# GBATZOLIS/conditional_score_diffusion

Hardware: AMD Instinct MI355X
Metric: images/sec for 1000-step PC sampling, ddpm_paired_SR3 score net of celebA_SR3_160 (BASELINE configs[1]), 160x160 (higher is better)
Workload: dtype f16x3 (every operand carried as hi + lo fp16 = 22 significand bits, 3 MFMAs per product, f32 accumulate; f32-class: the per-op test tolerance is the f32 kernel's, network error 1.9e-6 vs the reference); 1 GPU; BASELINE configs[1]: celebA_SR3_160 (ddpm_paired_SR3, nf=96, ch_mult (1,1,2,2,3,3), attn 20/10/5), 1000-step PC (reverse_diffusion + langevin, snr 0.15), batch 64 per GPU, random-init weights, synthetic LR inputs; images_per_gpu=64, global_batch=64, noise=on-device Philox4x32-10, precision_mode=fp16x3

## Files before the change

conditional_score_diffusion_amd/_lib.py:

```python
import ctypes
import os
import subprocess
import sys

_HERE = os.path.dirname(os.path.abspath(__file__))
LIB_PATH = os.environ.get('CSD_LIB_PATH', os.path.join(_HERE, 'libcsd_hip.so'))
CSRC = os.path.join(_HERE, 'csrc')

MAX_LEVELS = 8
MAX_ATTN = 8

ACT_IDS = {'none': 0, 'swish': 1, 'relu': 2, 'lrelu': 3, 'elu': 4}
PREC_IDS = {'fp32': 0, 'f32': 0, 'fp16x3': 1, 'fp16': 2, 'fp16f8': 3}


class UNetConfig(ctypes.Structure):
    _fields_ = [('arch', ctypes.c_int32), ('nf', ctypes.c_int32), ('n_levels', ctypes.c_int32),
                ('ch_mult', ctypes.c_int32 * MAX_LEVELS), ('num_res_blocks', ctypes.c_int32),
                ('n_attn', ctypes.c_int32), ('attn_resolutions', ctypes.c_int32 * MAX_ATTN),
                ('image_size', ctypes.c_int32), ('x_channels', ctypes.c_int32),
                ('y_channels', ctypes.c_int32), ('out_channels', ctypes.c_int32),
                ('resamp_with_conv', ctypes.c_int32), ('conditional', ctypes.c_int32),
                ('centered', ctypes.c_int32), ('act', ctypes.c_int32), ('precision', ctypes.c_int32),
                ('skip_rescale', ctypes.c_int32), ('progressive', ctypes.c_int32), ('progressive_input', ctypes.c_int32),
# ... 86 lines not shown
    'csd_fused_bias_act': (_i, [_vp, _vp, _vp, _vp, _i64, _i, _i64, _i, _i, _f, _f, _vp]),
    'csd_nearest_up2': (_i, [_vp, _vp, _i, _i, _i, _i, _vp]),
    'csd_timestep_embedding': (_i, [_vp, _vp, _i, _i, _vp]),
    'csd_conv_wgrad_scratch_bytes': (_sz, [_i, _i, _i, _i, _i, _i, _i, _i]),
    'csd_conv2d_wgrad': (_i, [_vp, _vp, _vp, _i, _i, _i, _i, _i, _i, _i, _i, _i, _vp, _vp]),
    'csd_groupnorm_act_backward': (_i, [_vp, _vp, _vp, _vp, _vp, _vp, _vp, _i, _i, _i, _i, _i, _f, _i, _vp]),
    'csd_attention_backward_scratch_bytes': (_sz, [_i, _i, _i, _i]),
    'csd_attention_backward': (_i, [_vp, _vp, _vp, _vp, _vp, _vp, _vp, _i, _i, _i, _i, _vp, _vp]),
    'csd_bgemm': (_i, [_vp, _vp, _vp, _i, _i, _i, _i64, _i64, _i64, _i64, _i64, _i64, _i, _i64, _i64, _i64, _f, _vp]),
    'csd_sum_inner': (_i, [_vp, _vp, _i64, _i64, _vp]),
    'csd_sum_rows': (_i, [_vp, _vp, _i, _i, _vp]),
    'csd_act': (_i, [_vp, _vp, _vp, _i, _i64, _vp]),
    'csd_mul': (_i, [_vp, _vp, _vp, _i64, _vp]),
    'csd_conv3x3_block_scratch_bytes': (_sz, [_i, _i]),
    'csd_conv3x3_block': (_i, [_vp, _vp, _vp, _vp, _vp, _vp, _vp, _i, _vp, _f, _vp, _vp, _i, _i, _i, _i, _i, _i, _i, _vp, _vp]),
    'csd_conv2d_ex': (_i, [_vp, _vp, _vp, _vp, _i, _i, _i, _i, _i, _i, _i, _i, _i, _i, _i, _vp, _vp]),
    'csd_conv2d_wgrad_ex': (_i, [_vp, _vp, _vp, _i, _i, _i, _i, _i, _i, _i, _i, _i, _i, _vp, _vp]),
    'csd_groupnorm_nhwc_scratch_bytes': (_sz, [_i, _i, _i]),
    'csd_groupnorm_act_nhwc': (_i, [_vp, _vp, _vp, _vp, _vp, _vp, _i, _i, _i, _i, _f, _i, _vp, _vp]),
    'csd_groupnorm_act_backward_nhwc': (_i, [_vp, _vp, _vp, _vp, _vp, _vp, _vp, _vp, _vp, _i, _i, _i, _i, _i, _i, _vp, _vp]),
    'csd_bias_add_nhwc': (_i, [_vp, _vp, _vp, _i, _i, _i, _vp]),
    'csd_sum_pixels_scratch_bytes': (_sz, [_i, _i, _i]),
    'csd_sum_pixels_nhwc': (_i, [_vp, _vp, _i, _i, _i, _vp, _vp]),
    'csd_zero_insert_odd_nhwc': (_i, [_vp, _vp, _i, _i, _i, _i, _vp]),
    'csd_sumpool2_nhwc': (_i, [_vp, _vp, _i, _i, _i, _i, _vp]),
    'csd_attention_nhwc': (_i, [_vp, _vp, _i, _i, _i, _vp]),
    'csd_attention_nhwc_prec': (_i, [_vp, _vp, _i, _i, _i, _i, _vp]),
    'csd_attention_backward_nhwc': (_i, [_vp, _vp, _vp, _i, _i, _i, _vp, _vp]),
    'csd_adam_step': (_i, [_vp, _vp, _vp, _vp, _vp, _vp, _i64, _i, _f, _f, _f, _f, _f, _f, _f, _vp]),
    'csd_global_norm_scratch_bytes': (_sz, []),
# ... 81 lines not shown
```

conditional_score_diffusion_amd/csrc/common.h:

```cpp
#pragma once
#include <hip/hip_runtime.h>
#include <stdint.h>
#include <stdio.h>
#include <string>

#include "../../include/csd.h"

#ifdef CSD_TUNE
#define CSD_TUNE_ENV(name) getenv(name)
#else
#define CSD_TUNE_ENV(name) (static_cast<const char*>(nullptr))
#endif

namespace csd {

void set_error(const char* fmt, ...);
const char* get_error();

#define CSD_CHECK_HIP(expr)                                                         \
  do {                                                                              \
    hipError_t _e = (expr);                                                         \
    if (_e != hipSuccess) {                                                         \
      csd::set_error("%s:%d: %s -> %s", __FILE__, __LINE__, #expr, hipGetErrorString(_e)); \
      return CSD_ERR_HIP;                                                           \
// ... 119 lines not shown
int conv16_plan_tiles(ConvPlan* p, int ns, int kcs = 1, bool lc = false);
size_t conv16_packed_bytes(const ConvPlan& p, int ns);
int conv16_pack_weight(const ConvPlan& p, int ns, const float* w, int layout, int cin_src, int cout_src,
                       int cout_off, void* wpack, hipStream_t s);
int conv16_launch(const ConvPlan& p, int ns, const ConvArgs& a, hipStream_t s, bool in16 = false);
bool conv16q_supported(const ConvPlan& p, int ns);
size_t conv16q_packed_bytes(const ConvPlan& p, int ns);
int conv16q_pack_weight(const ConvPlan& p, int ns, const float* w, int layout, int cin_src, int cout_src, int cout_off,
                        void* wpack, hipStream_t s);
int conv16q_plan_tiles(ConvPlan* p, int ns);
bool conv16q_up4_supported(const ConvPlan& p, int ns);
bool conv16q_up4_stats_ok(const ConvPlan& p);
size_t conv16q_up4_packed_bytes(const ConvPlan& p, int ns);
int conv16q_pack_weight_up4(const ConvPlan& p, int ns, const float* w, void* wpack, hipStream_t s);
int conv16q_launch(const ConvPlan& p, int ns, const ConvArgs& a, hipStream_t s, bool raw = false);
bool convff_supported(const ConvPlan& p, int ns);
size_t convff_packed_bytes(const ConvPlan& p, int ns);
int convff_pack_weight(const ConvPlan& p, int ns, const float* w, int layout, int cin_src, int cout_src, int cout_off,
                       void* wpack, hipStream_t s);
int convff_plan_tiles(ConvPlan* p, int ns);
bool convff_pipelined(const ConvPlan& p, int ns);
int convff_launch(const ConvPlan& p, int ns, const ConvArgs& a, hipStream_t s);
bool pw16_supported(const ConvPlan& p, int ns);
size_t pw16_packed_bytes(const ConvPlan& p, int ns);
int pw16_pack_weight(const ConvPlan& p, int ns, const float* w, int layout, int cin_src, int cout_src, int cout_off,
                     void* wpack, hipStream_t s);
int pw16_launch(const ConvPlan& p, int ns, const ConvArgs& a, hipStream_t s);
bool pw16_taps_supported(int cin, int cout, int ns);
int pw16_taps_cout(int cout);
int pw16_pack_weight_taps(const ConvPlan& p, int ns, const float* w, int cout, void* wpack, hipStream_t s);
// ... 103 lines not shown
```

conditional_score_diffusion_amd/csrc/conv_f16_q.hip:

```cpp
#include <stdlib.h>
#include <type_traits>

#include "conv_f16_kernel.h"

namespace csd {

typedef float floatx4q __attribute__((ext_vector_type(4)));
typedef unsigned int uint4q __attribute__((ext_vector_type(4)));

#define C16Q_THREADS 256

__device__ __forceinline__ double dpp_row16_sum(double v) {
#define CSD_DPP_STEP(CTRL)                                                                                   \
  {                                                                                                          \
    const int lo = __builtin_amdgcn_mov_dpp(__double2loint(v), CTRL, 0xF, 0xF, true);                        \
    const int hi = __builtin_amdgcn_mov_dpp(__double2hiint(v), CTRL, 0xF, 0xF, true);                        \
    v += __hiloint2double(hi, lo);                                                                           \
  }
  CSD_DPP_STEP(0xB1)
  CSD_DPP_STEP(0x4E)
  CSD_DPP_STEP(0x124)
  CSD_DPP_STEP(0x128)
#undef CSD_DPP_STEP
  return v;
}
__device__ __forceinline__ float dpp_row16_sum(float v) {
#define CSD_DPP_STEP_F(CTRL) v += __int_as_float(__builtin_amdgcn_mov_dpp(__float_as_int(v), CTRL, 0xF, 0xF, true));
  CSD_DPP_STEP_F(0xB1)
  CSD_DPP_STEP_F(0x4E)
  CSD_DPP_STEP_F(0x124)
  CSD_DPP_STEP_F(0x128)
#undef CSD_DPP_STEP_F
  return v;
}

typedef int int8q __attribute__((ext_vector_type(8)));

template <int MQ, int NS, bool MASK, int PWC, int S, int NTQ, bool F8, bool UP4 = false, bool RAW = false>
__global__ __launch_bounds__(C16Q_THREADS, 2) void conv_f16_q_kernel(const void* __restrict__ g_hi,
                                                                    const void* __restrict__ g_lo,
                                                                    const char* __restrict__ g_wpack,
                                                                    const Conv16KArgs k) {
  static_assert(!UP4 || (S == 1 && !F8), "the phase form is the stride-1 Upsample conv (a resampling conv: full split)");
  static_assert(!RAW || (NS == 2 && !F8), "the fp32-source form splits into two fp16 planes");
  constexpr int TAPS = UP4 ? 4 : 9, KS = UP4 ? 2 : 3, KCS = 2;
  constexpr int LO = 32 * KCS;
  constexpr int PSB = 32 * KCS * NS + 16;
  constexpr int NPIX = 2 * MQ * 16;
  constexpr int SPP = 2 * NS * KCS;
  constexpr int NU0 = (S == 2) ? ((NS == 2) ? 10 : 5) : ((NS == 2) ? 7 : 4);
  constexpr int NU = RAW ? 2 * ((NU0 + 1) / 2) : NU0;
  constexpr int rstride = PWC * PSB;
  constexpr int WSTEP = NTQ * NS * 1024;
  constexpr int GC = 32 * NTQ, HC = 16 * NTQ;
  extern __shared__ __attribute__((aligned(16))) char smem16[];

  const int tid = threadIdx.x;
#ifdef CSD_C16_TIMING
  int ts_n = 0;
#define Q_TSTAMP() do { if (k.a.dbg && tid == 0 && blockIdx.x < 4095 && ts_n < 8) k.a.dbg[blockIdx.x * 8 + ts_n++] = clock64(); } while (0)
#else
#define Q_TSTAMP() do { } while (0)
#endif
  Q_TSTAMP();
  const int lane = tid & 63;
  const int wave = __builtin_amdgcn_readfirstlane(tid >> 6);
  const int mi = wave >> 1, ni = wave & 1;
// ... 5 lines not shown
    const int xcd = bid & 7, slot = bid >> 3;
    const int q = nb >> 3, r = nb & 7;
    w = (xcd < r ? xcd * (q + 1) : r * (q + 1) + (xcd - r) * q) + slot;
  }
  const int ng = w % k.n_groups;
  const int tile4 = w / k.n_groups;
  const int ph = UP4 ? (tile4 & 3) : 0, pa = ph >> 1, pb = ph & 1;
  const int tile = UP4 ? (tile4 >> 2) : tile4;
  const int tile_y = tile / k.tiles_x;
  const int ov0 = tile_y * k.TH, ox0 = (tile - tile_y * k.tiles_x) * k.TW;
  const int Py = UP4 ? 1 - pa : ((S == 2) ? 0 : 1), Px = UP4 ? 1 - pb : ((S == 2) ? 0 : 1);
  const int prow0 = ov0 * S - Py, pcol0 = ox0 * S - Px;
  const int EH = (S == 2) ? k.IH : k.OH, EW = (S == 2) ? k.IW : k.OW;
  const int Cin = k.C0;
  const int npatch = k.PH * k.PW;
  const int patch_bytes = k.PH * PWC * PSB;
  int* const otab = reinterpret_cast<int*>(smem16 + patch_bytes);
  int* const btab = otab + NPIX;
  int* const vtab = btab + NPIX;
  int* const stab = vtab + NPIX;
  int* const dtab = stab + npatch;

  for (int m = tid; m < NPIX; m += C16Q_THREADS) {
    const int ty = m / k.TW, tx = m - ty * k.TW;
    const int ov = ov0 + ty, ox = ox0 + tx;
    const bool mv = (m < k.TH * k.TW) && (ov < k.B * k.OH) && (ox < k.OW);
    const int b = ov / k.OH, oy = ov - b * k.OH;
    unsigned vb = 0;
#pragma unroll
    for (int r = 0; r < KS; ++r) {
      const int iy = oy * S + r - Py, ix = ox * S + r - Px;
      vb |= ((mv && iy >= 0 && iy < EH) ? 1u : 0u) << r;
      vb |= ((mv && ix >= 0 && ix < EW) ? 1u : 0u) << (3 + r);
    }
    otab[m] = mv ? (UP4 ? (ov - ov0) * 4 * k.OW + 2 * ox : (ov - ov0) * k.OW + ox) : -1;
    btab[m] = mv ? b : 0;
    vtab[m] = (int)vb;
  }
  for (int pix = tid; pix < npatch; pix += C16Q_THREADS) {
    const int pr = pix / k.PW, pc = pix - pr * k.PW;
    const int vr = prow0 + pr, col = pcol0 + pc;
    const int img_lo = MASK ? 0 : (ov0 / k.OH) * EH;
    const int img_hi = MASK ? k.B * EH : img_lo + EH;
    const bool in = vr >= img_lo && vr < img_hi && col >= 0 && col < EW;
    const int sb = vr / EH, sr = vr - sb * EH;
    stab[pix] = in ? (sb * k.IH + (sr >> k.up)) * k.IW + (col >> k.up) : -1;
    dtab[pix] = (pr * PWC + pc) * PSB;
  }
  int base[MQ];
#pragma unroll
  for (int j = 0; j < MQ; ++j) {
    const int m = (mi * MQ + j) * 16 + l16;
    const int ty = m / k.TW, tx = m - ty * k.TW;
    base[j] = (m < k.TH * k.TW) ? ty * S * rstride + tx * S * PSB + kq * 16 : kq * 16;
  }
  __syncthreads();
  Q_TSTAMP();
  unsigned vbits[MQ];
  if (MASK) {
#pragma unroll
    for (int j = 0; j < MQ; ++j) vbits[j] = (unsigned)vtab[(mi * MQ + j) * 16 + l16];
  }

  const int total4 = RAW ? npatch * 2 * KCS : npatch * SPP;
  auto raw_load = [&](int e, int cb, int half) -> float4 {
    float4 v = make_float4(0.f, 0.f, 0.f, 0.f);
    if (e < total4) {
      const int pix = e / (2 * KCS), grp = e - pix * (2 * KCS);
      const int sp = stab[pix];
      if (sp >= 0) v = gload4f(static_cast<const float*>(g_hi) + (size_t)sp * Cin + cb + grp * 8 + half * 4);
    }
    return v;
  };
  auto raw_store = [&](int e, const float4& a, const float4& b) {
    if (e >= total4) return;
    const int pix = e / (2 * KCS), grp = e - pix * (2 * KCS);
    const float v[8] = {a.x, a.y, a.z, a.w, b.x, b.y, b.z, b.w};
    half8 h, l;
#pragma unroll
    for (int j = 0; j < 8; ++j) {
      h[j] = (_Float16)v[j];
      l[j] = (_Float16)(v[j] - (float)h[j]);
    }
    *reinterpret_cast<half8*>(smem16 + dtab[pix] + grp * 16) = h;
    *reinterpret_cast<half8*>(smem16 + dtab[pix] + LO + grp * 16) = l;
  };
  auto slot_load = [&](int e, int cb) -> float4 {
    float4 v = make_float4(0.f, 0.f, 0.f, 0.f);
    if (e < total4) {
      const int pix = e / SPP, sub = e - pix * SPP;
      const int sp = stab[pix];
      if (sp >= 0) {
        const int pl = sub / (2 * KCS), rest = sub - pl * (2 * KCS);
        const _Float16* plane = static_cast<const _Float16*>((NS == 2 && pl) ? g_lo : g_hi);
        v = gload4f(reinterpret_cast<const float*>(plane + (size_t)sp * Cin + cb + rest * 8));
      }
    }
    return v;
  };
  auto slot_store = [&](int e, const float4& v) {
    if (e >= total4) return;
    const int pix = e / SPP, sub = e - pix * SPP;
    const int pl = sub / (2 * KCS), rest = sub - pl * (2 * KCS);
    *reinterpret_cast<float4*>(smem16 + dtab[pix] + pl * LO + rest * 16) = v;
  };

  constexpr int BR = UP4 ? 2 : (NTQ == 1 && !F8 ? 9 : 3);
  const int nk32 = Cin / 32;
  const char* wstep = g_wpack + ((size_t)((UP4 ? ph * k.n_groups * 2 : 0) + ng * 2 + ni) * nk32 * TAPS) * WSTEP + lane * 16;
  constexpr int NP = F8 ? 1 : NS;
  half8 wreg[BR][NTQ][NP];
#pragma unroll
  for (int q = 0; q < BR - 1; ++q)
#pragma unroll
    for (int t = 0; t < NTQ; ++t)
#pragma unroll
      for (int p = 0; p < NP; ++p) wreg[q][t][p] = gload_h8(wstep + (size_t)q * WSTEP + (t * NS + p) * 1024);
  wstep += (size_t)(BR - 2) * WSTEP;
  const char* const w8base = g_wpack + ((size_t)(ng * 2 + ni) * nk32 * TAPS + (kq >> 1)) * WSTEP + (lane & 31) * 32 + 1024;
  int8q w8[1][NTQ];
  auto load_w8 = [&](int buf, int step) {
#pragma unroll
// ... 2 lines not shown
      const uint4q c = *reinterpret_cast<const uint4q*>(w8base + (size_t)step * WSTEP + t * NS * 1024 + 16);
      w8[buf][t] = int8q{(int)a.x, (int)a.y, (int)a.z, (int)a.w, (int)c.x, (int)c.y, (int)c.z, (int)c.w};
    }
  };
  if constexpr (F8) load_w8(0, 0);
  int base8[MQ];
#pragma unroll
  for (int j = 0; j < MQ; ++j) base8[j] = base[j] - kq * 16 + LO + (kq & 1) * 32;

  floatx4q acc[MQ][NTQ];
#pragma unroll
  for (int j = 0; j < MQ; ++j)
#pragma unroll
    for (int t = 0; t < NTQ; ++t) acc[j][t] = floatx4q{0.f, 0.f, 0.f, 0.f};

  {
    float4 v0[NU];
    if constexpr (RAW) {
#pragma unroll
      for (int j = 0; j < NU; ++j) v0[j] = raw_load((j >> 1) * C16Q_THREADS + tid, 0, j & 1);
#pragma unroll
      for (int j = 0; j < NU; j += 2) raw_store((j >> 1) * C16Q_THREADS + tid, v0[j], v0[j + 1]);
    } else {
#pragma unroll
      for (int j = 0; j < NU; ++j) v0[j] = slot_load(j * C16Q_THREADS + tid, 0);
#pragma unroll
      for (int j = 0; j < NU; ++j) slot_store(j * C16Q_THREADS + tid, v0[j]);
    }
  }
  __syncthreads();
  Q_TSTAMP();

  const int nstage = nk32;
  for (int stg = 0; stg < nstage; ++stg) {
    const bool more = stg + 1 < nstage;
    float4 sv[NU];
    if (more) {
#pragma unroll
      for (int j = 0; j < NU; ++j)
        sv[j] = RAW ? raw_load((j >> 1) * C16Q_THREADS + tid, (stg + 1) * 32, j & 1) : slot_load(j * C16Q_THREADS + tid, (stg + 1) * 32);
    }
#ifdef CSD_Q_RING
    constexpr int RING = CSD_Q_RING;
#else
    constexpr int RING = 2;
#endif
    half8 preg[RING][NP];
    auto load_frag = [&](int q) {
      const int tap_ = q / MQ, j_ = q % MQ;
      const char* p = smem16 + base[j_] + (tap_ / KS) * rstride + (tap_ % KS) * PSB;
#pragma unroll
      for (int pl = 0; pl < NP; ++pl) preg[q % RING][pl] = *reinterpret_cast<const half8*>(p + pl * LO);
    };
#pragma unroll
    for (int q = 0; q < RING - 1; ++q) load_frag(q);
#pragma unroll
    for (int tap = 0; tap < TAPS; ++tap) {
      const int bc = tap % BR, bn = (tap + BR - 1) % BR;
      const int r = tap / KS, sx = tap % KS;
      wstep += WSTEP;
#ifndef CSD_Q_ABLATE
#define CSD_Q_ABLATE 0
#endif
#pragma unroll
      for (int t = 0; t < ((CSD_Q_ABLATE & 1) ? 1 : NTQ); ++t)
// ... 44 lines not shown
              ok = ok && ((vbits[j] >> (tt / KS)) & 1u) && ((vbits[j] >> (3 + tt % KS)) & 1u);
            }
            const int8q b8 = int8q{ok ? (int)a.x : 0, ok ? (int)a.y : 0, ok ? (int)a.z : 0, ok ? (int)a.w : 0,
                                   ok ? (int)c.x : 0, ok ? (int)c.y : 0, ok ? (int)c.z : 0, ok ? (int)c.w : 0};
#pragma unroll
            for (int t = 0; t < NTQ; ++t)
              acc[j][t] = __builtin_amdgcn_mfma_scale_f32_16x16x128_f8f6f4(w8[wb][t], b8, acc[j][t], 0, 0, 0, 116, 0, 127);
          }
          const int nxt = t0 + 2 < TAPS ? stg * TAPS + t0 + 2 : (stg + 1) * TAPS;
          if (t0 + 2 < TAPS || more) load_w8(0, nxt);
        }
      }
    }
    static_assert(TAPS % BR == 0, "weight ring phase");
    Q_TSTAMP();
    if (more) {
      __syncthreads();
      if constexpr (RAW) {
#pragma unroll
        for (int j = 0; j < NU; j += 2) raw_store((j >> 1) * C16Q_THREADS + tid, sv[j], sv[j + 1]);
      } else {
#pragma unroll
        for (int j = 0; j < NU; ++j) slot_store(j * C16Q_THREADS + tid, sv[j]);
      }
      __syncthreads();
    }
  }

  constexpr unsigned OOB = 0x80000000u;
  constexpr int RSRC_FLAGS = 0x00020000;
  const float wunscale = 1.0f / C16_WSCALE;
// ... 246 lines not shown
    static const long min_wg = CSD_TUNE_ENV("CSD_Q_MINWG") ? atol(CSD_TUNE_ENV("CSD_Q_MINWG")) : 300;
    if (up4 && (long)OHt * OWt >= 1600) break;
    if (nwg >= min_wg || mq == 2) break;
  }
  CSD_REQUIRE(best_tw > 0, "conv16q: no feasible tile for OW=%d", p->OW);
  p->TW = best_tw; p->TH = best_th;
  p->PH = in_coord_k(p->TH, st, ks); p->PW = in_coord_k(p->TW, st, ks);
  p->tiles_x = cdiv(OWt, p->TW);
  p->tiles_y = cdiv(p->B * OHt, p->TH);
  p->MT = best_mq;
  p->lds_bytes = (size_t)p->PH * pitch(p->TW) * psb + (size_t)3 * 2 * best_mq * 16 * sizeof(int) +
                 (size_t)2 * p->PH * p->PW * sizeof(int);
  return CSD_OK;
}

template <int MQ, int NS, bool MASK, int PWC, int S, int NTQ, bool F8 = false, bool UP4 = false, bool RAW = false>
static int launch_q(const Conv16KArgs& k, size_t lds, hipStream_t s) {
  auto kern = conv_f16_q_kernel<MQ, NS, MASK, PWC, S, NTQ, F8, UP4, RAW>;
  static bool attr_set = false;
  if (!attr_set) {
    CSD_CHECK_HIP(hipFuncSetAttribute(reinterpret_cast<const void*>(kern), hipFuncAttributeMaxDynamicSharedMemorySize, 160 * 1024));
    attr_set = true;
  }
  hipLaunchKernelGGL(kern, dim3(k.nblocks), dim3(C16Q_THREADS), lds, s, static_cast<const void*>(k.a.src0),
                     static_cast<const void*>(k.a.src1), reinterpret_cast<const char*>(k.a.wpack), k);
  CSD_LAUNCH_CHECK();
  return CSD_OK;
}

template <int MQ, int NS, bool MASK, int PWC, int S, int NTQ, bool UP4>
static int launch_q_src(bool raw, const Conv16KArgs& k, size_t lds, hipStream_t s) {
  if constexpr (NS == 2 && NTQ >= 3) {
    if (raw) return launch_q<MQ, NS, MASK, PWC, S, NTQ, false, UP4, true>(k, lds, s);
  }
  if (raw) {
    set_error("conv16q: no fp32-source kernel for ns=%d NT=%d", NS, NTQ);
    return CSD_ERR_INVALID;
  }
  return launch_q<MQ, NS, MASK, PWC, S, NTQ, false, UP4, false>(k, lds, s);
}

int conv16q_launch(const ConvPlan& p, int ns, const ConvArgs& a, hipStream_t s, bool raw) {
  const bool up4 = p.up == 2;
  CSD_REQUIRE(up4 ? conv16q_up4_supported(p, ns) : conv16q_supported(p, ns), "conv16q: unsupported layer");
  CSD_REQUIRE(!a.out_nchw && a.nscale == nullptr && a.out_stride % 4 == 0 && a.out_coff % 4 == 0,
              "conv16q: NHWC fp32 output with 16-byte aligned rows, pre-normalised fp16 source");
// ... 12 lines not shown
      g_c16_dbg_n++;
    }
  }
#endif
  k.B = p.B; k.IH = p.IH; k.IW = p.IW; k.OH = p.OH; k.OW = p.OW;
  k.C0 = p.C0; k.C1 = 0; k.Cout = p.Cout;
  k.stride = p.stride; k.pad = p.stride == 2 ? 0 : 1; k.up = p.up;
  k.TH = p.TH; k.TW = p.TW; k.PH = p.PH; k.PW = p.PW;
  k.tiles_x = p.tiles_x; k.n_groups = p.n_groups;
  k.nblocks = p.tiles_x * p.tiles_y * p.n_groups * (up4 ? 4 : 1);
  if (up4) { k.OH = p.IH; k.OW = p.IW; k.up = 0; }
  k.nck = p.C0 / C16_KC;
  k.nw = 4;
  k.ntiles_n = p.Cout / 32;
  const bool mask = ((up4 ? p.IH : p.OH) % p.TH) != 0;
#define CSD_QU_CASE(MQ_, NS_, NTQ_)                                                              \
  if (up4 && p.MT == MQ_ && ns == NS_ && p.NT == NTQ_) {                                        \
    if (p.PW <= 24) {                                                                            \
      if (mask) return launch_q_src<MQ_, NS_, true, 24, 1, NTQ_, true>(raw, k, p.lds_bytes, s);    \
      return launch_q_src<MQ_, NS_, false, 24, 1, NTQ_, true>(raw, k, p.lds_bytes, s);             \
    }                                                                                            \
    if (mask) return launch_q_src<MQ_, NS_, true, 34, 1, NTQ_, true>(raw, k, p.lds_bytes, s);      \
    return launch_q_src<MQ_, NS_, false, 34, 1, NTQ_, true>(raw, k, p.lds_bytes, s);               \
  }
  CSD_QU_CASE(4, 2, 3) CSD_QU_CASE(2, 2, 3) CSD_QU_CASE(4, 1, 3) CSD_QU_CASE(2, 1, 3)
  CSD_QU_CASE(4, 2, 4) CSD_QU_CASE(2, 2, 4) CSD_QU_CASE(4, 1, 4) CSD_QU_CASE(2, 1, 4)
#undef CSD_QU_CASE
  CSD_REQUIRE(!up4, "conv16q: no phase kernel for MQ=%d ns=%d NT=%d", p.MT, ns, p.NT);
#define CSD_Q_CASE(MQ_, NS_, NTQ_)                                                  \
  if (p.MT == MQ_ && ns == NS_ && p.NT == NTQ_ && p.stride == 1) {                  \
    if (p.PW <= 24) {                                                               \
      if (mask) return launch_q_src<MQ_, NS_, true, 24, 1, NTQ_, false>(raw, k, p.lds_bytes, s);    \
      return launch_q_src<MQ_, NS_, false, 24, 1, NTQ_, false>(raw, k, p.lds_bytes, s);             \
    }                                                                               \
    if (mask) return launch_q_src<MQ_, NS_, true, 34, 1, NTQ_, false>(raw, k, p.lds_bytes, s);      \
    return launch_q_src<MQ_, NS_, false, 34, 1, NTQ_, false>(raw, k, p.lds_bytes, s);               \
  }                                                                                 \
  if (p.MT == MQ_ && ns == NS_ && p.NT == NTQ_ && p.stride == 2) {                  \
    if (p.PW <= 24) {                                                               \
      if (mask) return launch_q_src<MQ_, NS_, true, 24, 2, NTQ_, false>(raw, k, p.lds_bytes, s);    \
      return launch_q_src<MQ_, NS_, false, 24, 2, NTQ_, false>(raw, k, p.lds_bytes, s);             \
    }                                                                               \
    if (mask) return launch_q_src<MQ_, NS_, true, 34, 2, NTQ_, false>(raw, k, p.lds_bytes, s);      \
    return launch_q_src<MQ_, NS_, false, 34, 2, NTQ_, false>(raw, k, p.lds_bytes, s);               \
  }
#define CSD_Q8_CASE(MQ_, NTQ_)                                                         \
  if (p.MT == MQ_ && ns == 3 && p.NT == NTQ_ && p.stride == 1) {                     \
    if (p.PW <= 24) {                                                                \
      if (mask) return launch_q<MQ_, 2, true, 24, 1, NTQ_, true>(k, p.lds_bytes, s);  \
      return launch_q<MQ_, 2, false, 24, 1, NTQ_, true>(k, p.lds_bytes, s);           \
    }                                                                                \
    if (mask) return launch_q<MQ_, 2, true, 34, 1, NTQ_, true>(k, p.lds_bytes, s);    \
    return launch_q<MQ_, 2, false, 34, 1, NTQ_, true>(k, p.lds_bytes, s);             \
  }                                                                                  \
  if (p.MT == MQ_ && ns == 3 && p.NT == NTQ_ && p.stride == 2) {                     \
    if (p.PW <= 24) {                                                                \
      if (mask) return launch_q<MQ_, 2, true, 24, 2, NTQ_, true>(k, p.lds_bytes, s);  \
      return launch_q<MQ_, 2, false, 24, 2, NTQ_, true>(k, p.lds_bytes, s);           \
    }                                                                                \
// ... 15 lines not shown
```

conditional_score_diffusion_amd/csrc/ops_api.hip:

```cpp
#include <stdlib.h>
#include <string.h>

#include "common.h"

using namespace csd;

namespace {
inline int ceil8(int v) { return (v + 7) / 8 * 8; }
inline int ceil16(int v) { return (v + 15) / 16 * 16; }
inline size_t al64(size_t v) { return (v + 63) / 64 * 64; }
}

extern "C" size_t csd_groupnorm_scratch_bytes(int B, int C, int H, int W) {
  GNPlan g;
  if (gn_plan(&g, B, H * W, C, 0, 1)) return 0;
  const size_t t = (size_t)B * H * W * C;
  return (2 * al64(t) + 2 * al64((size_t)B * C)) * sizeof(float) + gn_partial_bytes(g) * 64 + 1024;
}

extern "C" int csd_groupnorm_act(const float* x, const float* gamma, const float* beta, float* y, int B, int C,
                                 int H, int W, int groups, float eps, int act, void* scratch, void* stream) {
  CSD_REQUIRE(x && gamma && beta && y && scratch, "groupnorm: null argument");
  hipStream_t s = (hipStream_t)stream;
  GNPlan g;
// ... 207 lines not shown
  memset(&p, 0, sizeof(p));
  p.B = B; p.IH = p.OH = H; p.IW = p.OW = W; p.C0 = C0; p.C1 = C1; p.Cout = Cout; p.taps = 9; p.stride = 1; p.pad = 1; p.up = 0;
  CSD_REQUIRE(convff_supported(p, ns), "conv3x3_block: unsupported shape (C %d+%d -> %d, %dx%d)", C0, C1, Cout, H, W);
  int rc = convff_plan_tiles(&p, ns);
  if (rc) return rc;
  void* wpack = reinterpret_cast<void*>((reinterpret_cast<uintptr_t>(scratch) + 255) & ~(uintptr_t)255);
  if ((rc = convff_pack_weight(p, ns, weight, 0, C0 + C1, Cout, 0, wpack, s))) return rc;
  ConvArgs a;
  memset(&a, 0, sizeof(a));
  a.src0 = x0; a.src1 = x1; a.wpack = static_cast<const float*>(wpack); a.bias = bias; a.temb = temb; a.res = res;
  a.nscale = nscale; a.nshift = nshift; a.out = y; a.temb_stride = temb_stride; a.out_stride = Cout; a.out_coff = 0;
  a.out_nchw = 0; a.act = CSD_ACT_SWISH; a.out_scale = out_scale; a.stats = stats; a.dbg = nullptr;
  return convff_launch(p, ns, a, s);
}

extern "C" size_t csd_attention_scratch_bytes(int B, int C, int H, int W) {
  const size_t L = (size_t)H * W;
  return (al64((size_t)B * L * 3 * C) + al64((size_t)B * L * C)) * sizeof(float) + 1024;
}

extern "C" int csd_attention(const float* q, const float* k, const float* v, float* out, int B, int C, int H, int W,
                             void* scratch, void* stream) {
  CSD_REQUIRE(q && k && v && out && scratch, "attention: null argument");
  hipStream_t s = (hipStream_t)stream;
  const int L = H * W;
  float* f = static_cast<float*>(scratch);
  float* qkv = f; f += al64((size_t)B * L * 3 * C);
  float* oh = f;
  int rc;
  if ((rc = nchw_to_nhwc_launch(q, qkv, B, C, L, C, 3 * C, s))) return rc;
// ... 29 lines not shown
```

conditional_score_diffusion_amd/ops.py:

```python
import torch

from . import _lib
from ._lib import check, current_stream, lib, ptr, require_gpu_tensor


def _scratch(nbytes, device):
    return torch.empty(max(int(nbytes), 256), dtype=torch.uint8, device=device)


def _c(t, name):
    require_gpu_tensor(t, name)
    return t.contiguous()


def groupnorm_act(x, gamma, beta, groups=32, eps=1e-6, act='none'):
    x, gamma, beta = _c(x, 'x'), _c(gamma, 'gamma'), _c(beta, 'beta')
    B, C, H, W = x.shape
    y = torch.empty_like(x)
    sc = _scratch(lib().csd_groupnorm_scratch_bytes(B, C, H, W), x.device)
    check(lib().csd_groupnorm_act(ptr(x), ptr(gamma), ptr(beta), ptr(y), B, C, H, W, groups, eps,
                                  _lib.ACT_IDS[act], ptr(sc), current_stream(x.device)), 'groupnorm_act')
    return y


# ... 56 lines not shown
    Cout = weight.shape[0]
    if tuple(weight.shape) != (Cout, C0 + C1, 3, 3):
        raise RuntimeError('conv3x3_block: weight %s does not match %d input channels' % (tuple(weight.shape), C0 + C1))
    opt = [None if t is None else _c(t, 't') for t in (bias, nscale, nshift, temb, res)]
    bias, nscale, nshift, temb, res = opt
    y = torch.empty(B, H, W, Cout, dtype=torch.float32, device=x0.device)
    stats = torch.empty(B * ((H + 15) // 16) * ((W + 15) // 16), Cout, 2, dtype=torch.float64, device=x0.device) if want_stats else None
    sc = _scratch(lib().csd_conv3x3_block_scratch_bytes(C0 + C1, Cout), x0.device)
    check(lib().csd_conv3x3_block(ptr(x0), ptr(x1), ptr(weight), ptr(bias), ptr(nscale), ptr(nshift), ptr(temb),
                                  temb.shape[1] if temb is not None else 0, ptr(res), float(out_scale), ptr(y), ptr(stats),
                                  B, C0, C1, Cout, H, W, _lib.PREC_IDS[precision], ptr(sc), current_stream(x0.device)),
          'conv3x3_block')
    return (y, stats) if want_stats else y


def attention(q, k, v):
    q, k, v = _c(q, 'q'), _c(k, 'k'), _c(v, 'v')
    B, C, H, W = q.shape
    out = torch.empty_like(q)
    sc = _scratch(lib().csd_attention_scratch_bytes(B, C, H, W), q.device)
    check(lib().csd_attention(ptr(q), ptr(k), ptr(v), ptr(out), B, C, H, W, ptr(sc), current_stream(q.device)),
          'attention')
    return out


def _upfirdn2d_raw(x, kernel, up, down, pad4):
    x, kernel = _c(x, 'x'), _c(kernel, 'kernel')
    N, C, H, W = x.shape
    kh, kw = kernel.shape
    (ux, uy), (dx, dy), (px0, px1, py0, py1) = up, down, pad4
# ... 172 lines not shown
```

include/csd.h:

```cpp
#ifndef CSD_H_
#define CSD_H_

#include <stddef.h>
#include <stdint.h>

#ifdef __cplusplus
extern "C" {
#endif

typedef enum csd_status {
  CSD_OK = 0,
  CSD_ERR_INVALID = -1,
  CSD_ERR_HIP = -2,
  CSD_ERR_STATE = -3,
  CSD_ERR_NOT_FOUND = -4,
  CSD_ERR_WORKSPACE = -5,
  CSD_ERR_NONFINITE = -6
} csd_status;

enum { CSD_ACT_NONE = 0, CSD_ACT_SWISH = 1, CSD_ACT_RELU = 2, CSD_ACT_LRELU = 3, CSD_ACT_ELU = 4 };

enum {
  CSD_PREC_F32 = 0,
  CSD_PREC_F16X3 = 1,
// ... 164 lines not shown
int csd_dropout(const float* x, float* out, float* mask, float p, uint64_t seed, uint64_t stream_id, int64_t n,
                void* stream);

int csd_adam_step(float* param, const float* grad, float* exp_avg, float* exp_avg_sq, float* ema,
                  const float* grad_norm, int64_t n, int step, float lr, float beta1, float beta2, float eps,
                  float weight_decay, float max_norm, float ema_decay, void* stream);
size_t csd_global_norm_scratch_bytes(void);
int csd_global_norm(const float* a, float* out, int64_t n, void* scratch, void* stream);
int csd_ema_update(float* ema, const float* param, int64_t n, float decay, void* stream);

size_t csd_conv3x3_block_scratch_bytes(int Cin, int Cout);
int csd_conv3x3_block(const float* x0, const float* x1, const float* weight, const float* bias, const float* nscale,
                      const float* nshift, const float* temb, int temb_stride, const float* res, float out_scale, float* y,
                      double* stats, int B, int C0, int C1, int Cout, int H, int W, int precision, void* scratch, void* stream);

int csd_conv2d_ex(const float* x, const float* weight, const float* bias, float* y, int B, int Cin, int Cout, int H, int W,
                  int ksize, int stride, int pad_mode, int up2, int precision, int layout, void* scratch, void* stream);
int csd_conv2d_wgrad_ex(const float* x, const float* dy, float* dw, int B, int Cin, int Cout, int H, int W, int ksize,
                        int stride, int pad_mode, int up2, int layout, void* scratch, void* stream);
size_t csd_groupnorm_nhwc_scratch_bytes(int B, int C, int HW);
int csd_groupnorm_act_nhwc(const float* x, const float* gamma, const float* beta, float* y, float* rs, float* ms, int B,
                           int C, int HW, int groups, float eps, int act, void* scratch, void* stream);
int csd_groupnorm_act_backward_nhwc(const float* x, const float* gamma, const float* beta, const float* rs, const float* ms,
                                    const float* dy, float* dx, float* dgamma_rows, float* dbeta_rows, int row_stride, int B, int C,
                                    int HW, int groups, int act, void* scratch, void* stream);
int csd_bias_add_nhwc(const float* x, const float* bias, float* out, int B, int HW, int C, void* stream);
size_t csd_sum_pixels_scratch_bytes(int B, int HW, int C);
int csd_sum_pixels_nhwc(const float* x, float* out, int B, int HW, int C, void* scratch, void* stream);
int csd_zero_insert_odd_nhwc(const float* dy, float* z, int B, int h, int w, int C, void* stream);
int csd_sumpool2_nhwc(const float* in, float* out, int B, int h, int w, int C, void* stream);
// ... 32 lines not shown
```

Measured before the change: 1.574 images/sec.

## Add multi-buffered chunked LDS schedule for small-map stride-1 fp16x3 convs

Adds a variant of the quad-split 3x3 conv kernel that loads four input-channel stages at a time into registers and stores them into a ring of eight LDS patch buffers. The kernel then needs one barrier per chunk instead of one per stage. It is chosen automatically when the workgroup count fits within the CU count and the ring fits in LDS, which targets the low-resolution levels where few workgroups run. The cost is one workgroup per CU and much more register and LDS use. A standalone API entry point is also added so the conv can be tested.

```diff
diff --git a/conditional_score_diffusion_amd/_lib.py b/conditional_score_diffusion_amd/_lib.py
--- a/conditional_score_diffusion_amd/_lib.py
+++ b/conditional_score_diffusion_amd/_lib.py
@@ -124,6 +124,9 @@
     'csd_mul': (_i, [_vp, _vp, _vp, _i64, _vp]),
     'csd_conv3x3_block_scratch_bytes': (_sz, [_i, _i]),
     'csd_conv3x3_block': (_i, [_vp, _vp, _vp, _vp, _vp, _vp, _vp, _i, _vp, _f, _vp, _vp, _i, _i, _i, _i, _i, _i, _i, _vp, _vp]),
+    'csd_conv3x3_quad_scratch_bytes': (_sz, [_i, _i, _i, _i, _i]),
+    'csd_conv3x3_quad_info': (_i, [_i, _i, _i, _i, _i, _i, ctypes.POINTER(_i)]),
+    'csd_conv3x3_quad': (_i, [_vp, _vp, _vp, _vp, _i, _vp, _f, _vp, _vp, _i, _i, _i, _i, _i, _i, _i, _vp, _vp]),
     'csd_conv2d_ex': (_i, [_vp, _vp, _vp, _vp, _i, _i, _i, _i, _i, _i, _i, _i, _i, _i, _i, _vp, _vp]),
     'csd_conv2d_wgrad_ex': (_i, [_vp, _vp, _vp, _i, _i, _i, _i, _i, _i, _i, _i, _i, _i, _vp, _vp]),
     'csd_groupnorm_nhwc_scratch_bytes': (_sz, [_i, _i, _i]),
diff --git a/conditional_score_diffusion_amd/csrc/common.h b/conditional_score_diffusion_amd/csrc/common.h
--- a/conditional_score_diffusion_amd/csrc/common.h
+++ b/conditional_score_diffusion_amd/csrc/common.h
@@ -157,6 +157,7 @@
 size_t conv16q_up4_packed_bytes(const ConvPlan& p, int ns);
 int conv16q_pack_weight_up4(const ConvPlan& p, int ns, const float* w, void* wpack, hipStream_t s);
 int conv16q_launch(const ConvPlan& p, int ns, const ConvArgs& a, hipStream_t s, bool raw = false);
+int conv16q_ring_chunk(const ConvPlan& p, int ns);
 bool convff_supported(const ConvPlan& p, int ns);
 size_t convff_packed_bytes(const ConvPlan& p, int ns);
 int convff_pack_weight(const ConvPlan& p, int ns, const float* w, int layout, int cin_src, int cout_src, int cout_off,
diff --git a/conditional_score_diffusion_amd/csrc/conv_f16_q.hip b/conditional_score_diffusion_amd/csrc/conv_f16_q.hip
--- a/conditional_score_diffusion_amd/csrc/conv_f16_q.hip
+++ b/conditional_score_diffusion_amd/csrc/conv_f16_q.hip
@@ -36,13 +36,27 @@
 
 typedef int int8q __attribute__((ext_vector_type(8)));
 
-template <int MQ, int NS, bool MASK, int PWC, int S, int NTQ, bool F8, bool UP4 = false, bool RAW = false>
-__global__ __launch_bounds__(C16Q_THREADS, 2) void conv_f16_q_kernel(const void* __restrict__ g_hi,
+template <int G>
+struct QRingCfg {
+  static constexpr int D = G > 0 ? 2 * G : 1;
+  static constexpr int WGS_PER_CU = G >= 3 ? 1 : 2;
+  static constexpr int LDS_CU = 160 * 1024;
+  static constexpr int LDS_BUDGET = LDS_CU / WGS_PER_CU;
+  static_assert(G == 0 || D >= 3, "a burst is stored while the stage before it may still be read: at least three buffers");
+  static_assert(LDS_BUDGET * WGS_PER_CU <= LDS_CU, "the co-resident workgroups share one CU's LDS");
+  static constexpr size_t tables(int npix, int npatch) { return (size_t)(3 * npix + 2 * npatch) * sizeof(int); }
+  static constexpr size_t bytes(int patch_bytes, int npix, int npatch) { return (size_t)D * patch_bytes + tables(npix, npatch); }
+  static constexpr bool fits(int patch_bytes, int npix, int npatch) { return bytes(patch_bytes, npix, npatch) <= (size_t)LDS_BUDGET; }
+};
+
+template <int MQ, int NS, bool MASK, int PWC, int S, int NTQ, bool F8, bool UP4 = false, bool RAW = false, int G = 0>
+__global__ __launch_bounds__(C16Q_THREADS, QRingCfg<G>::WGS_PER_CU) void conv_f16_q_kernel(const void* __restrict__ g_hi,
                                                                     const void* __restrict__ g_lo,
                                                                     const char* __restrict__ g_wpack,
                                                                     const Conv16KArgs k) {
   static_assert(!UP4 || (S == 1 && !F8), "the phase form is the stride-1 Upsample conv (a resampling conv: full split)");
   static_assert(!RAW || (NS == 2 && !F8), "the fp32-source form splits into two fp16 planes");
+  static_assert(G == 0 || (S == 1 && !UP4 && !F8), "the small-map schedule covers the stride-1 3x3 forms");
   constexpr int TAPS = UP4 ? 4 : 9, KS = UP4 ? 2 : 3, KCS = 2;
   constexpr int LO = 32 * KCS;
   constexpr int PSB = 32 * KCS * NS + 16;
@@ -50,7 +64,8 @@
   constexpr int SPP = 2 * NS * KCS;
   constexpr int NU0 = (S == 2) ? ((NS == 2) ? 10 : 5) : ((NS == 2) ? 7 : 4);
   constexpr int NU = RAW ? 2 * ((NU0 + 1) / 2) : NU0;
-  constexpr int rstride = PWC * PSB;
+  const int pitch = G > 0 ? k.PW : PWC;
+  const int rstride = pitch * PSB;
   constexpr int WSTEP = NTQ * NS * 1024;
   constexpr int GC = 32 * NTQ, HC = 16 * NTQ;
   extern __shared__ __attribute__((aligned(16))) char smem16[];
@@ -86,8 +101,8 @@
   const int EH = (S == 2) ? k.IH : k.OH, EW = (S == 2) ? k.IW : k.OW;
   const int Cin = k.C0;
   const int npatch = k.PH * k.PW;
-  const int patch_bytes = k.PH * PWC * PSB;
-  int* const otab = reinterpret_cast<int*>(smem16 + patch_bytes);
+  const int patch_bytes = k.PH * pitch * PSB;
+  int* const otab = reinterpret_cast<int*>(smem16 + QRingCfg<G>::D * patch_bytes);
   int* const btab = otab + NPIX;
   int* const vtab = btab + NPIX;
   int* const stab = vtab + NPIX;
@@ -117,7 +132,7 @@
     const bool in = vr >= img_lo && vr < img_hi && col >= 0 && col < EW;
     const int sb = vr / EH, sr = vr - sb * EH;
     stab[pix] = in ? (sb * k.IH + (sr >> k.up)) * k.IW + (col >> k.up) : -1;
-    dtab[pix] = (pr * PWC + pc) * PSB;
+    dtab[pix] = (pr * pitch + pc) * PSB;
   }
   int base[MQ];
 #pragma unroll
@@ -144,7 +159,7 @@
     }
     return v;
   };
-  auto raw_store = [&](int e, const float4& a, const float4& b) {
+  auto raw_store = [&](int e, const float4& a, const float4& b, int sbuf = 0) {
     if (e >= total4) return;
     const int pix = e / (2 * KCS), grp = e - pix * (2 * KCS);
     const float v[8] = {a.x, a.y, a.z, a.w, b.x, b.y, b.z, b.w};
@@ -154,8 +169,8 @@
       h[j] = (_Float16)v[j];
       l[j] = (_Float16)(v[j] - (float)h[j]);
     }
-    *reinterpret_cast<half8*>(smem16 + dtab[pix] + grp * 16) = h;
-    *reinterpret_cast<half8*>(smem16 + dtab[pix] + LO + grp * 16) = l;
+    *reinterpret_cast<half8*>(smem16 + sbuf + dtab[pix] + grp * 16) = h;
+    *reinterpret_cast<half8*>(smem16 + sbuf + dtab[pix] + LO + grp * 16) = l;
   };
   auto slot_load = [&](int e, int cb) -> float4 {
     float4 v = make_float4(0.f, 0.f, 0.f, 0.f);
@@ -170,14 +185,17 @@
     }
     return v;
   };
-  auto slot_store = [&](int e, const float4& v) {
+  auto slot_store = [&](int e, const float4& v, int sbuf = 0) {
     if (e >= total4) return;
     const int pix = e / SPP, sub = e - pix * SPP;
     const int pl = sub / (2 * KCS), rest = sub - pl * (2 * KCS);
-    *reinterpret_cast<float4*>(smem16 + dtab[pix] + pl * LO + rest * 16) = v;
+    *reinterpret_cast<float4*>(smem16 + sbuf + dtab[pix] + pl * LO + rest * 16) = v;
   };
 
-  constexpr int BR = UP4 ? 2 : (NTQ == 1 && !F8 ? 9 : 3);
+#ifndef CSD_Q_RING_BR9
+#define CSD_Q_RING_BR9 0
+#endif
+  constexpr int BR = UP4 ? 2 : (((NTQ == 1 && !F8) || (G >= 3 && CSD_Q_RING_BR9)) ? 9 : 3);
   const int nk32 = Cin / 32;
   const char* wstep = g_wpack + ((size_t)((UP4 ? ph * k.n_groups * 2 : 0) + ng * 2 + ni) * nk32 * TAPS) * WSTEP + lane * 16;
   constexpr int NP = F8 ? 1 : NS;
@@ -210,7 +228,38 @@
 #pragma unroll
     for (int t = 0; t < NTQ; ++t) acc[j][t] = floatx4q{0.f, 0.f, 0.f, 0.f};
 
-  {
+  const int nstage = nk32;
+  float4 cv[G > 0 ? G : 1][NU];
+  auto chunk_load = [&](int c) {
+#pragma unroll
+    for (int g = 0; g < G; ++g) {
+      const int st = c * G + g;
+      if (st < nstage) {
+#pragma unroll
+        for (int j = 0; j < NU; ++j)
+          cv[g][j] = RAW ? raw_load((j >> 1) * C16Q_THREADS + tid, st * 32, j & 1) : slot_load(j * C16Q_THREADS + tid, st * 32);
+      }
+    }
+  };
+  auto chunk_store = [&](int c) {
+#pragma unroll
+    for (int g = 0; g < G; ++g) {
+      if (c * G + g < nstage) {
+        const int sb = ((c & 1) * G + g) * patch_bytes;
+        if constexpr (RAW) {
+#pragma unroll
+          for (int j = 0; j < NU; j += 2) raw_store((j >> 1) * C16Q_THREADS + tid, cv[g][j], cv[g][j + 1], sb);
+        } else {
+#pragma unroll
+          for (int j = 0; j < NU; ++j) slot_store(j * C16Q_THREADS + tid, cv[g][j], sb);
+        }
+      }
+    }
+  };
+  if constexpr (G > 0) {
+    chunk_load(0);
+    chunk_store(0);
+  } else {
     float4 v0[NU];
     if constexpr (RAW) {
 #pragma unroll
@@ -227,11 +276,15 @@
   __syncthreads();
   Q_TSTAMP();
 
-  const int nstage = nk32;
   for (int stg = 0; stg < nstage; ++stg) {
     const bool more = stg + 1 < nstage;
-    float4 sv[NU];
-    if (more) {
+    float4 sv[G > 0 ? 1 : NU];
+    int sbuf = 0;
+    const int chunk = G > 0 ? stg / (G > 0 ? G : 1) : 0, cg = G > 0 ? stg - chunk * G : 0;
+    if constexpr (G > 0) {
+      if (cg == 0) chunk_load(chunk + 1);
+      sbuf = ((chunk & 1) * G + cg) * patch_bytes;
+    } else if (more) {
 #pragma unroll
       for (int j = 0; j < NU; ++j)
         sv[j] = RAW ? raw_load((j >> 1) * C16Q_THREADS + tid, (stg + 1) * 32, j & 1) : slot_load(j * C16Q_THREADS + tid, (stg + 1) * 32);
@@ -244,7 +297,7 @@
     half8 preg[RING][NP];
     auto load_frag = [&](int q) {
       const int tap_ = q / MQ, j_ = q % MQ;
-      const char* p = smem16 + base[j_] + (tap_ / KS) * rstride + (tap_ % KS) * PSB;
+      const char* p = smem16 + sbuf + base[j_] + (tap_ / KS) * rstride + (tap_ % KS) * PSB;
 #pragma unroll
       for (int pl = 0; pl < NP; ++pl) preg[q % RING][pl] = *reinterpret_cast<const half8*>(p + pl * LO);
     };
@@ -319,7 +372,12 @@
     }
     static_assert(TAPS % BR == 0, "weight ring phase");
     Q_TSTAMP();
-    if (more) {
+    if constexpr (G > 0) {
+      if (more && cg == G - 1) {
+        chunk_store(chunk + 1);
+        __syncthreads();
+      }
+    } else if (more) {
       __syncthreads();
       if constexpr (RAW) {
 #pragma unroll
@@ -596,9 +654,9 @@
   return CSD_OK;
 }
 
-template <int MQ, int NS, bool MASK, int PWC, int S, int NTQ, bool F8 = false, bool UP4 = false, bool RAW = false>
+template <int MQ, int NS, bool MASK, int PWC, int S, int NTQ, bool F8 = false, bool UP4 = false, bool RAW = false, int G = 0>
 static int launch_q(const Conv16KArgs& k, size_t lds, hipStream_t s) {
-  auto kern = conv_f16_q_kernel<MQ, NS, MASK, PWC, S, NTQ, F8, UP4, RAW>;
+  auto kern = conv_f16_q_kernel<MQ, NS, MASK, PWC, S, NTQ, F8, UP4, RAW, G>;
   static bool attr_set = false;
   if (!attr_set) {
     CSD_CHECK_HIP(hipFuncSetAttribute(reinterpret_cast<const void*>(kern), hipFuncAttributeMaxDynamicSharedMemorySize, 160 * 1024));
@@ -610,8 +668,32 @@
   return CSD_OK;
 }
 
+int conv16q_ring_chunk(const ConvPlan& p, int ns) {
+  if (ns != 2 || p.stride != 1 || p.up != 0 || getenv("CSD_Q_OLD_SCHEDULE")) return 0;
+  static const int ncu = [] {
+    int dev = 0, n = 0;
+    if (hipGetDevice(&dev) != hipSuccess || hipDeviceGetAttribute(&n, hipDeviceAttributeMultiprocessorCount, dev) != hipSuccess) n = 0;
+    return n;
+  }();
+  const int psb = 32 * 2 * 2 + 16, npatch = p.PH * p.PW, npix = 2 * p.MT * 16;
+  const long nwg = (long)p.tiles_x * p.tiles_y * p.n_groups;
+  if (nwg <= ncu && QRingCfg<4>::fits(npatch * psb, npix, npatch)) return 4;
+  return 0;
+}
+
 template <int MQ, int NS, bool MASK, int PWC, int S, int NTQ, bool UP4>
-static int launch_q_src(bool raw, const Conv16KArgs& k, size_t lds, hipStream_t s) {
+static int launch_q_src(bool raw, int ring, const Conv16KArgs& k, size_t lds, hipStream_t s) {
+  if constexpr (NS == 2 && S == 1 && !UP4) {
+    const int npatch = k.PH * k.PW, pb = npatch * (32 * 2 * NS + 16), npix = 2 * MQ * 16;
+    if constexpr (NTQ >= 3) {
+      if (ring == 4 && raw) return launch_q<MQ, NS, MASK, 24, 1, NTQ, false, false, true, 4>(k, QRingCfg<4>::bytes(pb, npix, npatch), s);
+    }
+    if (ring == 4 && !raw) return launch_q<MQ, NS, MASK, 24, 1, NTQ, false, false, false, 4>(k, QRingCfg<4>::bytes(pb, npix, npatch), s);
+    if (ring) {
+      set_error("conv16q: no small-map kernel for chunk %d NT=%d raw=%d", ring, NTQ, (int)raw);
+      return CSD_ERR_INVALID;
+    }
+  }
   if constexpr (NS == 2 && NTQ >= 3) {
     if (raw) return launch_q<MQ, NS, MASK, PWC, S, NTQ, false, UP4, true>(k, lds, s);
   }
@@ -654,14 +736,15 @@
   k.nw = 4;
   k.ntiles_n = p.Cout / 32;
   const bool mask = ((up4 ? p.IH : p.OH) % p.TH) != 0;
+  const int ring = conv16q_ring_chunk(p, ns);
 #define CSD_QU_CASE(MQ_, NS_, NTQ_)                                                              \
   if (up4 && p.MT == MQ_ && ns == NS_ && p.NT == NTQ_) {                                        \
     if (p.PW <= 24) {                                                                            \
-      if (mask) return launch_q_src<MQ_, NS_, true, 24, 1, NTQ_, true>(raw, k, p.lds_bytes, s);    \
-      return launch_q_src<MQ_, NS_, false, 24, 1, NTQ_, true>(raw, k, p.lds_bytes, s);             \
+      if (mask) return launch_q_src<MQ_, NS_, true, 24, 1, NTQ_, true>(raw, 0, k, p.lds_bytes, s);    \
+      return launch_q_src<MQ_, NS_, false, 24, 1, NTQ_, true>(raw, 0, k, p.lds_bytes, s);             \
     }                                                                                            \
-    if (mask) return launch_q_src<MQ_, NS_, true, 34, 1, NTQ_, true>(raw, k, p.lds_bytes, s);      \
-    return launch_q_src<MQ_, NS_, false, 34, 1, NTQ_, true>(raw, k, p.lds_bytes, s);               \
+    if (mask) return launch_q_src<MQ_, NS_, true, 34, 1, NTQ_, true>(raw, 0, k, p.lds_bytes, s);      \
+    return launch_q_src<MQ_, NS_, false, 34, 1, NTQ_, true>(raw, 0, k, p.lds_bytes, s);               \
   }
   CSD_QU_CASE(4, 2, 3) CSD_QU_CASE(2, 2, 3) CSD_QU_CASE(4, 1, 3) CSD_QU_CASE(2, 1, 3)
   CSD_QU_CASE(4, 2, 4) CSD_QU_CASE(2, 2, 4) CSD_QU_CASE(4, 1, 4) CSD_QU_CASE(2, 1, 4)
@@ -670,19 +753,19 @@
 #define CSD_Q_CASE(MQ_, NS_, NTQ_)                                                  \
   if (p.MT == MQ_ && ns == NS_ && p.NT == NTQ_ && p.stride == 1) {                  \
     if (p.PW <= 24) {                                                               \
-      if (mask) return launch_q_src<MQ_, NS_, true, 24, 1, NTQ_, false>(raw, k, p.lds_bytes, s);    \
-      return launch_q_src<MQ_, NS_, false, 24, 1, NTQ_, false>(raw, k, p.lds_bytes, s);             \
+      if (mask) return launch_q_src<MQ_, NS_, true, 24, 1, NTQ_, false>(raw, ring, k, p.lds_bytes, s);    \
+      return launch_q_src<MQ_, NS_, false, 24, 1, NTQ_, false>(raw, ring, k, p.lds_bytes, s);             \
     }                                                                               \
-    if (mask) return launch_q_src<MQ_, NS_, true, 34, 1, NTQ_, false>(raw, k, p.lds_bytes, s);      \
-    return launch_q_src<MQ_, NS_, false, 34, 1, NTQ_, false>(raw, k, p.lds_bytes, s);               \
+    if (mask) return launch_q_src<MQ_, NS_, true, 34, 1, NTQ_, false>(raw, ring, k, p.lds_bytes, s);      \
+    return launch_q_src<MQ_, NS_, false, 34, 1, NTQ_, false>(raw, ring, k, p.lds_bytes, s);               \
   }                                                                                 \
   if (p.MT == MQ_ && ns == NS_ && p.NT == NTQ_ && p.stride == 2) {                  \
     if (p.PW <= 24) {                                                               \
-      if (mask) return launch_q_src<MQ_, NS_, true, 24, 2, NTQ_, false>(raw, k, p.lds_bytes, s);    \
-      return launch_q_src<MQ_, NS_, false, 24, 2, NTQ_, false>(raw, k, p.lds_bytes, s);             \
+      if (mask) return launch_q_src<MQ_, NS_, true, 24, 2, NTQ_, false>(raw, ring, k, p.lds_bytes, s);    \
+      return launch_q_src<MQ_, NS_, false, 24, 2, NTQ_, false>(raw, ring, k, p.lds_bytes, s);             \
     }                                                                               \
-    if (mask) return launch_q_src<MQ_, NS_, true, 34, 2, NTQ_, false>(raw, k, p.lds_bytes, s);      \
-    return launch_q_src<MQ_, NS_, false, 34, 2, NTQ_, false>(raw, k, p.lds_bytes, s);               \
+    if (mask) return launch_q_src<MQ_, NS_, true, 34, 2, NTQ_, false>(raw, ring, k, p.lds_bytes, s);      \
+    return launch_q_src<MQ_, NS_, false, 34, 2, NTQ_, false>(raw, ring, k, p.lds_bytes, s);               \
   }
 #define CSD_Q8_CASE(MQ_, NTQ_)                                                         \
   if (p.MT == MQ_ && ns == 3 && p.NT == NTQ_ && p.stride == 1) {                     \
diff --git a/conditional_score_diffusion_amd/csrc/ops_api.hip b/conditional_score_diffusion_amd/csrc/ops_api.hip
--- a/conditional_score_diffusion_amd/csrc/ops_api.hip
+++ b/conditional_score_diffusion_amd/csrc/ops_api.hip
@@ -245,6 +245,62 @@
   return convff_launch(p, ns, a, s);
 }
 
+static int quad_api_plan(ConvPlan* p, int B, int Cin, int Cout, int H, int W, int groups32) {
+  memset(p, 0, sizeof(*p));
+  p->B = B; p->IH = p->OH = H; p->IW = p->OW = W; p->C0 = Cin; p->C1 = 0; p->Cout = Cout; p->taps = 9; p->stride = 1; p->pad = 1; p->up = 0;
+  p->qnt = groups32 ? 1 : 0;
+  CSD_REQUIRE(B >= 1 && H >= 1 && W >= 1 && Cin >= 32 && conv16q_supported(*p, 2), "conv3x3_quad: unsupported shape (C %d -> %d, %dx%d)", Cin, Cout, H, W);
+  return conv16q_plan_tiles(p, 2);
+}
+
+extern "C" size_t csd_conv3x3_quad_scratch_bytes(int B, int Cin, int Cout, int H, int W) {
+  ConvPlan p;
+  if (quad_api_plan(&p, B, Cin, Cout, H, W, 0)) return 0;
+  p.qnt = 1;
+  const size_t w1 = Cout % 32 == 0 ? conv16q_packed_bytes(p, 2) : 0;
+  p.qnt = 0;
+  const size_t w0 = conv16q_packed_bytes(p, 2);
+  return (w0 > w1 ? w0 : w1) + (size_t)B * H * W * Cin * 4 + 4096;
+}
+
+extern "C" int csd_conv3x3_quad_info(int B, int Cin, int Cout, int H, int W, int groups32, int* info) {
+  CSD_REQUIRE(info, "conv3x3_quad_info: null argument");
+  ConvPlan p;
+  int rc = quad_api_plan(&p, B, Cin, Cout, H, W, groups32);
+  if (rc) return rc;
+  info[0] = p.tiles_x * p.tiles_y * 2;
+  info[1] = (H % p.TH) != 0;
+  info[2] = p.tiles_x * p.tiles_y * p.n_groups;
+  info[3] = conv16q_ring_chunk(p, 2);
+  return CSD_OK;
+}
+
+extern "C" int csd_conv3x3_quad(const float* x, const float* weight, const float* bias, const float* temb, int temb_stride,
+                                const float* res, float out_scale, float* y, double* stats, int B, int Cin, int Cout, int H, int W,
+                                int groups32, int raw, void* scratch, void* stream) {
+  CSD_REQUIRE(x && weight && y && scratch, "conv3x3_quad: null argument");
+  hipStream_t s = (hipStream_t)stream;
+  ConvPlan p;
+  int rc = quad_api_plan(&p, B, Cin, Cout, H, W, groups32);
+  if (rc) return rc;
+  CSD_REQUIRE(!stats || H % p.TH == 0, "conv3x3_quad: statistics need tiles that lie inside one sample");
+  CSD_REQUIRE(!raw || p.NT >= 3, "conv3x3_quad: the fp32-source form has three or four cout tiles per N half");
+  CSD_REQUIRE(!bias || (reinterpret_cast<uintptr_t>(bias) & 15) == 0, "conv3x3_quad: bias must be 16-byte aligned");
+  char* const wp = reinterpret_cast<char*>((reinterpret_cast<uintptr_t>(scratch) + 255) & ~(uintptr_t)255);
+  char* const hi = wp + ((conv16q_packed_bytes(p, 2) + 255) & ~(size_t)255);
+  char* const lo = hi + (size_t)B * H * W * Cin * 2;
+  if (!raw && (rc = gn_apply16_launch(x, nullptr, Cin, 0, nullptr, nullptr, hi, lo, B, H * W, CSD_ACT_NONE, s))) return rc;
+  if ((rc = conv16q_pack_weight(p, 2, weight, 0, Cin, Cout, 0, wp, s))) return rc;
+  ConvArgs a;
+  memset(&a, 0, sizeof(a));
+  a.src0 = raw ? x : reinterpret_cast<const float*>(hi);
+  a.src1 = raw ? nullptr : reinterpret_cast<const float*>(lo);
+  a.wpack = reinterpret_cast<const float*>(wp);
+  a.bias = bias; a.res = res; a.temb = temb; a.temb_stride = temb_stride;
+  a.out = y; a.out_stride = Cout; a.out_nchw = 0; a.out_scale = out_scale; a.stats = stats;
+  return conv16q_launch(p, 2, a, s, raw != 0);
+}
+
 extern "C" size_t csd_attention_scratch_bytes(int B, int C, int H, int W) {
   const size_t L = (size_t)H * W;
   return (al64((size_t)B * L * 3 * C) + al64((size_t)B * L * C)) * sizeof(float) + 1024;
diff --git a/conditional_score_diffusion_amd/ops.py b/conditional_score_diffusion_amd/ops.py
--- a/conditional_score_diffusion_amd/ops.py
+++ b/conditional_score_diffusion_amd/ops.py
@@ -94,6 +94,31 @@
     return (y, stats) if want_stats else y
 
 
+def conv3x3_quad_info(B, Cin, Cout, H, W, groups32=False):
+    import ctypes
+    info = (ctypes.c_int * 4)()
+    check(lib().csd_conv3x3_quad_info(B, Cin, Cout, H, W, int(bool(groups32)), info), 'conv3x3_quad_info')
+    return {'stat_rows': info[0], 'straddles': bool(info[1]), 'workgroups': info[2], 'chunk': info[3]}
+
+
+def conv3x3_quad(x, weight, bias=None, temb=None, res=None, out_scale=1.0, groups32=False, raw=False, want_stats=False):
+    x, weight = _c(x, 'x'), _c(weight, 'weight')
+    B, H, W, Cin = x.shape
+    Cout = weight.shape[0]
+    if tuple(weight.shape) != (Cout, Cin, 3, 3):
+        raise RuntimeError('conv3x3_quad: weight %s does not match %d input channels' % (tuple(weight.shape), Cin))
+    bias, temb, res = [None if t is None else _c(t, 't') for t in (bias, temb, res)]
+    y = torch.empty(B, H, W, Cout, dtype=torch.float32, device=x.device)
+    stats = None
+    if want_stats:
+        stats = torch.empty(conv3x3_quad_info(B, Cin, Cout, H, W, groups32)['stat_rows'], Cout, 2, dtype=torch.float64, device=x.device)
+    sc = _scratch(lib().csd_conv3x3_quad_scratch_bytes(B, Cin, Cout, H, W), x.device)
+    check(lib().csd_conv3x3_quad(ptr(x), ptr(weight), ptr(bias), ptr(temb), temb.shape[1] if temb is not None else 0, ptr(res),
+                                 float(out_scale), ptr(y), ptr(stats), B, Cin, Cout, H, W, int(bool(groups32)), int(bool(raw)),
+                                 ptr(sc), current_stream(x.device)), 'conv3x3_quad')
+    return (y, stats) if want_stats else y
+
+
 def attention(q, k, v):
     q, k, v = _c(q, 'q'), _c(k, 'k'), _c(v, 'v')
     B, C, H, W = q.shape
diff --git a/include/csd.h b/include/csd.h
--- a/include/csd.h
+++ b/include/csd.h
@@ -202,6 +202,12 @@
                       const float* nshift, const float* temb, int temb_stride, const float* res, float out_scale, float* y,
                       double* stats, int B, int C0, int C1, int Cout, int H, int W, int precision, void* scratch, void* stream);
 
+size_t csd_conv3x3_quad_scratch_bytes(int B, int Cin, int Cout, int H, int W);
+int csd_conv3x3_quad_info(int B, int Cin, int Cout, int H, int W, int groups32, int* info);
+int csd_conv3x3_quad(const float* x, const float* weight, const float* bias, const float* temb, int temb_stride, const float* res,
+                     float out_scale, float* y, double* stats, int B, int Cin, int Cout, int H, int W, int groups32, int raw,
+                     void* scratch, void* stream);
+
 int csd_conv2d_ex(const float* x, const float* weight, const float* bias, float* y, int B, int Cin, int Cout, int H, int W,
                   int ksize, int stride, int pad_mode, int up2, int precision, int layout, void* scratch, void* stream);
 int csd_conv2d_wgrad_ex(const float* x, const float* dy, float* dw, int B, int Cin, int Cout, int H, int W, int ksize,
```

Result: no change. 1.566 images/sec (-0.5%).
